# shaygong322/Mujoco-LIP-MPC-Simulation

Hardware: AMD Instinct MI355X
Metric: MPC solves/sec (batched scenarios), N=3 horizon 5-obstacle, 1->8 MI355X (higher is better)
Workload: dtype f64

## Files before the change

### mujoco-lip-mpc-simulation_amd/csrc/alipmpc.hip

```cpp
#include <hip/hip_runtime.h>

#include <atomic>
#include <cmath>
#include <cstdint>
#include <cstdio>
#include <cstdlib>
#include <cstring>
#include <map>
#include <mutex>
#include <string>
#include <type_traits>
#include <unordered_map>
#include <vector>

#include "../../include/alipmpc.h"

#ifndef ALIP_PART
#define ALIP_PART_HOST 1
#define ALIP_PART_N(k) 1
#else
#define ALIP_PART_HOST (ALIP_PART == 0)
#define ALIP_PART_N(k) (ALIP_PART == (k))
#endif

// ... 191 lines not shown
    static constexpr int NCP = 16 * NT;
    static constexpr int nu = 5 * N;
    static constexpr int NTU = (nu + 15) / 16;
    static constexpr int NCPU = 16 * NTU;
    static constexpr int NG = 8 * (N + 1);
    static constexpr int KLD = NCP + 1;
};

__device__ __forceinline__ int lane_id() { return threadIdx.x & (WAVE - 1); }

__device__ __forceinline__ void wave_sync()
{
    __builtin_amdgcn_wave_barrier();
    asm volatile("" ::: "memory");
}

__device__ __forceinline__ int rfl(int x) { return __builtin_amdgcn_readfirstlane(x); }
#define RELAUNDER(x) asm volatile("" : "+v"(x))

__device__ __forceinline__ double uni(double v)
{
    const int lo = __builtin_amdgcn_readfirstlane(__double2loint(v));
    const int hi = __builtin_amdgcn_readfirstlane(__double2hiint(v));
    return __hiloint2double(hi, lo);
}

__device__ __forceinline__ double bcast(double v, int src)
{
    int lo = __builtin_amdgcn_readlane(__double2loint(v), src);
    int hi = __builtin_amdgcn_readlane(__double2hiint(v), src);
    return __hiloint2double(hi, lo);
}

template <int CTRL>
__device__ __forceinline__ double dpp(double v)
{
    int lo = __builtin_amdgcn_update_dpp(0, __double2loint(v), CTRL, 0xF, 0xF, false);
    int hi = __builtin_amdgcn_update_dpp(0, __double2hiint(v), CTRL, 0xF, 0xF, false);
    return __hiloint2double(hi, lo);
}
__device__ __forceinline__ void swap16(double v, double& a, double& b)
{
    auto lo = __builtin_amdgcn_permlane16_swap((unsigned)__double2loint(v), (unsigned)__double2loint(v), false, false);
    auto hi = __builtin_amdgcn_permlane16_swap((unsigned)__double2hiint(v), (unsigned)__double2hiint(v), false, false);
    a = __hiloint2double((int)hi[0], (int)lo[0]);
    b = __hiloint2double((int)hi[1], (int)lo[1]);
}
__device__ __forceinline__ void swap32(double v, double& a, double& b)
{
    auto lo = __builtin_amdgcn_permlane32_swap((unsigned)__double2loint(v), (unsigned)__double2loint(v), false, false);
    auto hi = __builtin_amdgcn_permlane32_swap((unsigned)__double2hiint(v), (unsigned)__double2hiint(v), false, false);
    a = __hiloint2double((int)hi[0], (int)lo[0]);
    b = __hiloint2double((int)hi[1], (int)lo[1]);
}

__device__ __forceinline__ float uni(float v)
{
    return __int_as_float(__builtin_amdgcn_readfirstlane(__float_as_int(v)));
}
__device__ __forceinline__ float bcast(float v, int src)
{
    return __int_as_float(__builtin_amdgcn_readlane(__float_as_int(v), src));
}
template <int CTRL>
__device__ __forceinline__ float dpp(float v)
{
    return __int_as_float(__builtin_amdgcn_update_dpp(0, __float_as_int(v), CTRL, 0xF, 0xF, false));
}
__device__ __forceinline__ void swap16(float v, float& a, float& b)
{
    auto x = __builtin_amdgcn_permlane16_swap((unsigned)__float_as_int(v), (unsigned)__float_as_int(v), false, false);
    a = __int_as_float((int)x[0]);
    b = __int_as_float((int)x[1]);
}
__device__ __forceinline__ void swap32(float v, float& a, float& b)
{
    auto x = __builtin_amdgcn_permlane32_swap((unsigned)__float_as_int(v), (unsigned)__float_as_int(v), false, false);
    a = __int_as_float((int)x[0]);
    b = __int_as_float((int)x[1]);
}

struct OpAdd {
    template <class T>
    __device__ T operator()(T a, T b) const { return a + b; }
};
struct OpMax {
    template <class T>
    __device__ T operator()(T a, T b) const { return fmax(a, b); }
};
struct OpMin {
    template <class T>
    __device__ T operator()(T a, T b) const { return fmin(a, b); }
};

template <class T, class Op>
__device__ __forceinline__ T wreduce(T v, Op op)
{
    v = op(v, dpp<0xB1>(v));
    v = op(v, dpp<0x4E>(v));
    v = op(v, dpp<0x141>(v));
    v = op(v, dpp<0x140>(v));
    T a, b;
    swap16(v, a, b);
    v = op(a, b);
    swap32(v, a, b);
    return uni(op(a, b));
}
template <class T>
__device__ __forceinline__ T wsum(T v) { return wreduce(v, OpAdd()); }
template <class T>
__device__ __forceinline__ T wmax(T v) { return wreduce(v, OpMax()); }
template <class T>
__device__ __forceinline__ T wmin(T v) { return wreduce(v, OpMin()); }
template <class T>
__device__ __forceinline__ void wsum2(T& a, T& b)
{
    a = wsum(a);
    b = wsum(b);
}
template <class T>
__device__ __forceinline__ T gsum(T v)
{
    T a, b;
    swap16(v, a, b);
    v = a + b;
    swap32(v, a, b);
    return a + b;
}


__device__ __forceinline__ void ld4(const double* p, double& a, double& b, double& c, double& d)
{
    const double2* q = reinterpret_cast<const double2*>(p);
    const double2 x = q[0], y = q[1];
    a = x.x; b = x.y; c = y.x; d = y.y;
}
__device__ __forceinline__ void ld4(const float* p, float& a, float& b, float& c, float& d)
{
    const float4 x = *reinterpret_cast<const float4*>(p);
// ... 211 lines not shown
}

__device__ __forceinline__ int fexp2(double x) { return __builtin_amdgcn_frexp_exp(x); }
__device__ __forceinline__ int fexp2(float x) { return __builtin_amdgcn_frexp_expf(x); }

__device__ __forceinline__ double rsqrt_nr(double d)
{
    double y = __builtin_amdgcn_rsq(d);
    const double h = 0.5 * d;
    y = y * fma(-h * y, y, 1.5);
    y = y * fma(-h * y, y, 1.5);
    return y;
}
__device__ __forceinline__ double rcp_nr(double x)
{
    double y = __builtin_amdgcn_rcp(x);
    double e = fma(-x, y, 1.0);
    y = fma(y, e, y);
    e = fma(-x, y, 1.0);
    return fma(y, e, y);
}
__device__ __forceinline__ float rsqrt_nr(float d)
{
    float y = __builtin_amdgcn_rsqf(d);
    return y * fmaf(-0.5f * d * y, y, 1.5f);
}
__device__ __forceinline__ float rcp_nr(float x)
{
    float y = __builtin_amdgcn_rcpf(x);
    return fmaf(y, fmaf(-x, y, 1.0f), y);
}

#include "fastmath.inc"

template <int N, class WT>
__device__ void prologue(const KP& P, const WT& w, const typename WT::real* G, const double* E,
                         long long b, double& gxg, double& gyg, int& legv, double& uj)
{
    using D = Dim<N>;
    const int lane = lane_id();
    const double* x0 = P.x0 + 5 * b;
    legv = P.leg[b];
    const int ncr = P.nc[b];
    const int ner = P.ne ? P.ne[b] : 0;
    double x0v0 = x0[0], x0v1 = x0[1];
    double g0 = P.goal[2 * b], g1 = P.goal[2 * b + 1];
    {
        bool valid = lane < ncr && lane < P.nc_max;
        double c0 = 0, c1 = 0, c2 = 0;
        if (valid) {
            const double* c = P.cir + ((size_t)b * P.nc_max + lane) * 3;
            c0 = c[0]; c1 = c[1]; c2 = c[2];
        }
        double d = (x0v0 - c0) * (x0v0 - c0) + (x0v1 - c1) * (x0v1 - c1) - c2 * c2;
        bool keep = valid && (!P.select_obs || d <= P.detect_r2);
        unsigned long long m = __ballot(keep);
        int pos = __builtin_popcountll(m & ((1ull << lane) - 1ull));
        if (keep) {
            w.obs[3 * pos + 0] = c0;
            w.obs[3 * pos + 1] = c1;
            w.obs[3 * pos + 2] = c2;
        }
        if (lane == 0) w.nsel[0] = __builtin_popcountll(m);
    }
    if (P.ne_max > 0) {
        bool valid = lane < ner && lane < P.ne_max;
// ... 113 lines not shown
__device__ __forceinline__ bool gj_lds(R* M, int lane)
{
    constexpr int NE = n * (n + 1), Q = (NE + WAVE - 1) / WAVE;
    int ei[Q], ej[Q];
#pragma unroll
    for (int q = 0; q < Q; ++q) {
        const int e = lane + WAVE * q;
        ei[q] = e < NE ? e / (n + 1) : n;
        ej[q] = e < NE ? e - (e / (n + 1)) * (n + 1) : n;
    }
#pragma unroll 1
    for (int p = 0; p < n; ++p) {
        const R d = M[p * LD + p];
        R mip[Q], mpj[Q], mij[Q];
#pragma unroll
        for (int q = 0; q < Q; ++q) {
            mip[q] = M[ei[q] * LD + p];
            mpj[q] = M[p * LD + ej[q]];
            mij[q] = M[ei[q] * LD + ej[q]];
        }
        if (!(d > R(0))) return false;
        const R inv = rcp_nr(d);
#pragma unroll
        for (int q = 0; q < Q; ++q) {
            const R f = mpj[q] * inv;
            const R upd = ei[q] == p ? f : fma(-mip[q], f, mij[q]);
            M[ei[q] * LD + ej[q]] = ej[q] > p ? upd : mij[q];
        }
        wave_sync();
    }
    return true;
}

template <int n, class R>
__device__ __forceinline__ bool gj_regs(R (&a)[n + 1], int lane)
{
#pragma unroll
    for (int p = 0; p < n; ++p) {
        const R d = bcast(a[p], p);
        if (!(d > R(0))) return false;
        const R m = lane == p ? R(0) : a[p] * rcp_nr(d);
#pragma unroll
        for (int j = p + 1; j <= n; ++j) a[j] = fma(-m, bcast(a[j], p), a[j]);
    }
    R dg = a[0];
#pragma unroll
    for (int i = 1; i < n; ++i) dg = lane == i ? a[i] : dg;
    a[n] = a[n] * rcp_nr(dg);
    return true;
}

template <int n, int LDK, int LD, class R>
__device__ __forceinline__ void gj_fill(const R* K, R* M, int lane, R dw)
{
    constexpr int NE = n * (n + 1), Q = (NE + WAVE - 1) / WAVE;
#pragma unroll
    for (int q = 0; q < Q; ++q) {
        const int e = lane + WAVE * q;
        const int i = e < NE ? e / (n + 1) : n, j = e < NE ? e - (e / (n + 1)) * (n + 1) : n;
        const R v = e < NE ? K[i * LDK + j] : R(0);
        M[i * LD + j] = v + (i == j && e < NE ? dw : R(0));
    }
}
template <int n, int LD, class R>
__device__ __forceinline__ void gj_zero(R* M, int lane)
{
    constexpr int NE = n * (n + 1), Q = (NE + WAVE - 1) / WAVE;
#pragma unroll
    for (int q = 0; q < Q; ++q) {
        const int e = lane + WAVE * q;
        const int i = e < NE ? e / (n + 1) : n, j = e < NE ? e - (e / (n + 1)) * (n + 1) : n;
        M[i * LD + j] = R(0);
    }
}

template <int N, class R>
struct WSS {
    typedef R real;
    R* V;
    R* Vt;
    R* dV;
    R* CT;
// ... 753 lines not shown
#pragma unroll
                for (int T = 0; T < NT; ++T) {
                    const int cc = 16 * T + col;
                    const R j = ca.x * G[gen_i(pk, 0) * NCP + cc] + ca.y * G[gen_i(pk, 1) * NCP + cc] +
                                     cb.x * G[gen_i(pk, 2) * NCP + cc] + cb.y * G[gen_i(pk, 3) * NCP + cc];
                    gl[T] += j * y;
                    if constexpr (JC) jv[JC ? s : 0][T] = j;
                }
            }
#pragma unroll
            for (int T = 0; T < NT; ++T) gl[T] = gsum(gl[T]);
            STAMP(1);
            RELANE();
            R ru = R(0.0);
#pragma unroll
            for (int T = 0; T < NT; ++T)
                if (g4 == 0 && 16 * T + col < n) ru = fmax(ru, fabs(gl[T]));
            R rcm = R(0.0), nz = R(0.0), whi = -INFINITY, wlo = INFINITY;
#pragma unroll
            for (int q = 0; q < RPL; ++q) {
                const R dl = sr[q] - cl[q], du = cu[q] - sr[q];
                if (rtype[q] < R_NONE) rcm = fmax(rcm, fabs(cr[q] - sr[q]));
                nz += fabs(zl[q]) + fabs(zu[q]);
                if (HL(q)) {
                    whi = fmax(whi, dl * zl[q]);
                    wlo = fmin(wlo, dl * zl[q]);
                }
                if (HU(q)) {
                    whi = fmax(whi, du * zu[q]);
                    wlo = fmin(wlo, du * zu[q]);
                }
            }
            nz = wsum(nz);
            const R sd = uni(div100(fmax(R(100.0), rcp_div(nz, w.cst[K_MACT] + n))));
            const R sc = uni(div100(fmax(R(100.0), rcp_div(nz, fmax(R(1.0), w.cst[K_NBL])))));
            const R base_err = wmax(fmax(rcp_div(ru, sd), rcm));
            whi = wmax(whi);
            wlo = wmin(wlo);
            const bool anyw = whi >= wlo;
            const R comp0 = anyw ? fmax(fabs(whi), fabs(wlo)) : R(0.0);
            e0 = uni(fmax(base_err, rcp_div(comp0, sc)));
            if (rfl(P.goal_abort)) {
                bool at_goal = false;
#pragma unroll
                for (int q = 0; q < RPL; ++q) {
                    const R dxg = CK.gxg - rv[q][0], dyg = CK.gyg - rv[q][1];
                    at_goal |= rtype[q] == R_OBJ && dxg * dxg + dyg * dyg == R(0);
                }
                if (__ballot(at_goal) != 0ull) {
                    fail_it = it + FAIL_GOAL;
                    it_end = it;
                    break;
                }
            }
            if (e0 <= w.cst[K_TOL]) {
                status = 0;
                break;
            }
            if (it >= it_end) break;
            const R mu_min = w.cst[K_TOL] / R(11.0);
            const R mu_prev = mu;
            for (int t = 0; t < 8; ++t) {
                const R cm = anyw ? fmax(fabs(whi - mu), fabs(wlo - mu)) : R(0.0);
                if (fmax(base_err, rcp_div(cm, sc)) <= R(10.0) * mu && mu > mu_min)
                    mu = uni(fmax(mu_min, fmin(R(0.2) * mu, mu * sqrt(mu))));
                else
                    break;
            }
            if (mu != mu_prev) nf = 0;
            break;
        }
// ... 93 lines not shown
                }
            }
#pragma unroll
            for (int T = 0; T < NT; ++T) rhsc[T] = gsum(pw[T]);
#pragma unroll
            for (int i = 0; i < 4; ++i) {
                const int row = Mfma<R>::row(g4, i);
                w.K[row * KLD + col] = acc[0][0][i] + acc[1][0][i];
                if constexpr (NT == 2) {
                    const R k1 = acc[0][1][i] + acc[1][1][i];
                    w.K[row * KLD + 16 + col] = k1;
                    w.K[(16 + col) * KLD + row] = k1;
                    w.K[(16 + row) * KLD + 16 + col] = acc[0][2][i] + acc[1][2][i];
                }
            }
        }
        wave_sync();
        STAMP(4);
        RELANE();
        R xv;
        bool fact_ok = true;
        {
            R rhs_l = R(0.0);
#pragma unroll
            for (int T = 0; T < NT; ++T) rhs_l = (lane < n && (lane >> 4) == T) ? rhsc[T] : rhs_l;
            if constexpr (GJ && GJ_REGS) {
                R a[n + 1];
                auto fill = [&](R dw) {
#pragma unroll
                    for (int j = 0; j < n; ++j) a[j] = (lane < n ? w.K[lane * KLD + j] : R(0.0)) + (lane == j ? dw : R(0.0));
                    a[n] = rhs_l + R(0.0);
                };
                fill(R(0));
                if (!gj_regs<n>(a, lane)) {
                    R dw = dw_last == R(0.0) ? R(1e-4) : fmax(R(1e-20), dw_last / R(3.0));
                    for (;;) {
                        fill(dw);
                        if (gj_regs<n>(a, lane)) break;
                        dw *= dw_last == R(0.0) ? R(100.0) : R(8.0);
                        if (dw > R(sizeof(R) == 8 ? 1e40 : 1e30)) {
                            fact_ok = false;
                            break;
                        }
                    }
                    dw_last = uni(dw);
                }
                xv = lane < n ? a[n] : R(0.0);
            } else if constexpr (GJ) {
                if (lane < n) w.K[lane * KLD + n] = rhs_l;
                wave_sync();
                gj_fill<n, KLD, GJLD>(w.K, w.S, lane, R(0));
                wave_sync();
                if (!gj_lds<n, GJLD>(w.S, lane)) {
                    R dw = dw_last == R(0.0) ? R(1e-4) : fmax(R(1e-20), dw_last / R(3.0));
                    for (;;) {
                        gj_fill<n, KLD, GJLD>(w.K, w.S, lane, dw);
                        wave_sync();
                        if (gj_lds<n, GJLD>(w.S, lane)) break;
                        dw *= dw_last == R(0.0) ? R(100.0) : R(8.0);
                        if (dw > R(sizeof(R) == 8 ? 1e40 : 1e30)) {
                            fact_ok = false;
                            break;
                        }
                    }
                    dw_last = uni(dw);
                }
                xv = lane < n ? w.S[lane * GJLD + n] : R(0.0);
            } else {
                R a[n];
                R myidg = R(1.0);
#pragma unroll
// ... 11 lines not shown
                            fact_ok = false;
                            break;
                        }
                    }
                    dw_last = uni(dw);
                }
                R acc = R(0.0), yv = R(0.0);
#pragma unroll
                for (int k = 0; k < n; ++k) {
                    const R yk = bcast((rhs_l - acc) * myidg, k);
                    yv = lane == k ? yk : yv;
                    acc += lane > k ? a[k] * yk : R(0.0);
                }
                wave_sync();
                if (lane < n) {
#pragma unroll
                    for (int j = 0; j < n; ++j) w.K[lane * KLD + j] = j <= lane ? a[j] : R(0.0);
                }
                wave_sync();
                acc = R(0.0);
                xv = R(0.0);
#pragma unroll
                for (int i = n - 1; i >= 0; --i) {
                    const R xi = bcast((yv - acc) * myidg, i);
                    xv = lane == i ? xi : xv;
                    acc += lane < i ? w.K[i * KLD + (lane & 31)] * xi : R(0.0);
                }
            }
        }
        STAMP(5);
        RELANE();
        {
            R v = R(0.0);
#pragma unroll
            for (int j = 0; j < n; ++j)
                v += G[(lane < NG ? lane : 0) * NCP + j] * (GJ && !GJ_REGS ? w.S[j * GJLD + n] : bcast(xv, j));
            dvme = lane < NG && fact_ok ? v : R(0.0);
            if (lane < NG) w.dV[lane] = dvme;
        }
        wave_sync();
        if constexpr (GJ && !GJ_REGS) gj_zero<n, GJLD>(w.S, lane);
        if (!fact_ok && fail_it < 0) {
            fail_it = it;
            it_end = it + 1;
        }
        RELANE();
        R dS[RPL], dZl[RPL], dZu[RPL];
        R ap = R(1.0), az = R(1.0), theta = R(0.0), sl = R(0.0), jdv[RPL];
#pragma unroll
        for (int q = 0; q < RPL; ++q) {
            const int r = lane + WAVE * q;
#pragma unroll
            for (int i = 0; i < 4; ++i) rdv[q][i] = w.dV[gen_i(rg[q], i)];
            R jd = R(0.0);
            if (r < mo4) {
                struct { R x, y; } ca, cb;
                ld4(w.rcoef + 4 * r, ca.x, ca.y, cb.x, cb.y);
                jd = ca.x * rdv[q][0] + ca.y * rdv[q][1] + cb.x * rdv[q][2] + cb.y * rdv[q][3];
            }
            jdv[q] = jd;
            dS[q] = rtype[q] < R_NONE ? jd + rcv[q] : R(0.0);
            dZl[q] = HL(q) ? mu * idl[q] - zl[q] - zl[q] * idl[q] * dS[q] : R(0.0);
            dZu[q] = HU(q) ? mu * idu[q] - zu[q] + zu[q] * idu[q] * dS[q] : R(0.0);
            const R dl = sr[q] - cl[q], du = cu[q] - sr[q];
            const R ids = rcp_nr(dS[q]);
            if (HL(q) && dS[q] < 0) ap = fmin(ap, -tau * dl * ids);
            if (HU(q) && dS[q] > 0) ap = fmin(ap, tau * du * ids);
            if (HL(q) && dZl[q] < 0) az = fmin(az, -tau * zl[q] * rcp_nr(dZl[q]));
            if (HU(q) && dZu[q] < 0) az = fmin(az, -tau * zu[q] * rcp_nr(dZu[q]));
            theta += fabs(rcv[q]);
            sl += (HL(q) ? dS[q] * idl[q] : R(0.0)) - (HU(q) ? dS[q] * idu[q] : R(0.0));
        }
        ap = wmin(ap);
        az = wmin(az);
        theta = theta_ok ? theta_c : wsum(theta);
        const R gdv = obj_sum<N, RPL>(jdv, mr4);
        sl = wsum(sl);
        const R phi = uni(f_cur - mu * lsum_cur);
        const R gphi = uni(gdv - mu * sl);
        const R lsw = uni(gphi < 0 ? sth * llog(theta) - sph * llog(-gphi) : R(0.0));
        R amin;
        if (gphi < 0) {
            amin = fmin(gth, gph * theta / -gphi);
            if (theta <= w.cst[K_THMIN]) amin = fmin(amin, exp(lsw));
        } else {
            amin = gth;
        }
        amin *= gal;
        amin = uni(amin > R(0) ? amin : R(8.673617379884035e-19));
        STAMP(6);
        R a = ap;
        R la = uni(llog(ap));
        bool accepted = false, ftype = false;
        R ctr[RPL], ta0[RPL], ta1[RPL];
        R ft = R(0.0), lgt = R(0.0), tht_acc = R(0.0);
        bool redo = false;
        for (;;) {
            R am = a, lam = la;
            if (!(TM && redo))
                for (int t = 0; t < -1 - tm; ++t) {
                    am = uni(am * R(0.5));
                    lam = uni(lam - R(M_LN2));
                }
            const bool valid = am >= amin;
            bool acc_m = false, fty_m = false;
            if (valid) {
                WSTAMP_TRIAL;
                RELANE();
                R tht = R(0.0);
                ft = R(0.0);
                lgt = R(0.0);
                bool bad = false;
#pragma unroll
                for (int q = 0; q < RPL; ++q) {
                    R vt[4];
#pragma unroll
                    for (int i = 0; i < 4; ++i) vt[i] = fma(am, rdv[q][i], rv[q][i]);
                    R o[6];
#pragma unroll
                    for (int i = 0; i < 6; ++i) o[i] = w.obs6[6 * roi[q] + i];
                    row_trans(rtype[q], vt, w.cst[K_GXG], w.cst[K_GYG], ta0[q], ta1[q]);
                    ctr[q] = row_value(rtype[q], rk[q], vt, ta0[q], ta1[q], o, CK);
                    const R st = sr[q] + am * dS[q];
                    if (rtype[q] < R_NONE) tht += fabs(ctr[q] - st);

                    const R d1 = st - cl[q], d2 = cu[q] - st;
                    if (HL(q) && !(d1 > 0)) bad = true;
                    if (HU(q) && !(d2 > 0)) bad = true;
                    lgt += llog(HL(q) ? (HU(q) ? d1 * d2 : d1) : (HU(q) ? d2 : R(1.0)));
                }
                tht = wsum(tht);
                ft = obj_sum<N, RPL>(ctr, mr4);
                lgt = wsum(lgt);
                const bool anybad = __ballot(bad) != 0ull;
                const R pht = anybad ? INFINITY : ft - mu * lgt;
                bool ok = isfinite(pht) && tht < w.cst[K_THMAX];
                if (ok) {
                    const bool b0 = lane < nf && !(tht < fth0 || pht < fph0);
                    const bool b1 = lane + WAVE < nf && !(tht < fth1 || pht < fph1);
                    ok = __ballot(b0 || b1) == 0ull;
                }
                if (ok) {
                    const bool switching = gphi < 0 && lam > lsw;
                    if (switching && theta <= w.cst[K_THMIN]) {
                        if (pht <= phi + eta * am * gphi) {
                            acc_m = true;
                            fty_m = true;
                        }
                    } else if (tht <= (1 - gth) * theta || pht <= phi - gph * theta) {
                        acc_m = true;
                        fty_m = false;
                    }
                }
                tht_acc = tht;
            }
            if (TM && redo) {
                accepted = true;
                break;
            }
            if (!TM || tm >= 0) {
                if (!valid) break;
                if (acc_m) {
                    accepted = true;
                    ftype = fty_m;
                    break;
                }
// ... 2596 lines not shown
    using L = SweepL<NC, FEN>;
    auto kern = sweep_kernel<NC, FEN, CH, WPG>;
    const size_t smem = sizeof(double) * ((size_t)L::GL + (size_t)WPG * (CH / 2) * L::SLOTD);
    set_smem((const void*)kern, smem);
    const unsigned res = resident_blocks((const void*)kern, smem, WAVE * WPG);
    const long long per = (long long)CH * WPG;
    const unsigned need = (unsigned)((P.B + per - 1) / per);
    const unsigned grid = res > 0 && res < need ? res : (need > 0 ? need : 1u);
    hipLaunchKernelGGL(kern, dim3(grid), dim3(WAVE * WPG), smem, st, P);
}
template <int NC, bool FEN>
void launch_sweep_s(const KP& P, hipStream_t st)
{
    const char* se = getenv("ALIPMPC_SWEEP_SHAPE");
    const int shape = se ? atoi(se) : SWEEP_SHAPE_DEFAULT;
    if (shape == 641)
        launch_sweep_t<NC, FEN, 64, 1>(P, st);
    else
        launch_sweep_t<NC, FEN, 32, 2>(P, st);
}
hipError_t launch_sweep(int nc, bool fen, const KP& P, hipStream_t st)
{
#define SWCASE(K)                                              \
    case K:                                                    \
        fen ? launch_sweep_s<K, true>(P, st) : launch_sweep_s<K, false>(P, st); \
        break;
    switch (nc) {
        SWCASE(0) SWCASE(1) SWCASE(2) SWCASE(3) SWCASE(4) SWCASE(5) SWCASE(6)
    default:
        return hipErrorInvalidValue;
    }
#undef SWCASE
    return hipGetLastError();
}
#endif

}

#if ALIP_PART_HOST
#include "scenes.inc"
#include "dataset.inc"

namespace {

using namespace alip;

struct Handle {
    alipmpc_cfg cfg;
    int device = 0;
    int N = 3, n = 9, NG = 32, NCP = 16, NCPU = 16, rps = 0, m_max = 0, mr4 = 0;
    int rps_s = 0, m_s = 0, mr4_s = 0, mo4 = 0;
    double* dGp = nullptr;
    double* dEp = nullptr;
    double* dGu = nullptr;
    double* dEu = nullptr;
    double* dlk = nullptr;
    float* dlkf = nullptr;
    int lane_nct = -1;
    int sweep_nc = -1;
    static constexpr unsigned NQ = 64;
    uint32_t* dq = nullptr;
    mutable std::atomic<unsigned> qi{0};
    void* stage = nullptr;
    size_t stage_bytes = 0;
    void* rstage = nullptr;
    size_t rstage_bytes = 0;
// ... 1465 lines not shown
    return ALIPMPC_OK;
}

#ifdef ALIP_STAMPS
int alipmpc_dbg_stamps(unsigned long long* out, int reset)
{
    if (hipMemcpyFromSymbol(out, HIP_SYMBOL(alip::g_stamps), sizeof(unsigned long long) * alip::NSTAMP) != hipSuccess)
        return -1;
    if (reset) {
        unsigned long long z[alip::NSTAMP] = {};
        if (hipMemcpyToSymbol(HIP_SYMBOL(alip::g_stamps), z, sizeof(z)) != hipSuccess) return -1;
    }
    return alip::NSTAMP;
}
#endif

#ifdef ALIP_WSTAMP
int alipmpc_dbg_wstamps(unsigned long long* out, long long slots)
{
    if (slots > alip::WSTAMP_CAP) slots = alip::WSTAMP_CAP;
    if (hipDeviceSynchronize() != hipSuccess) return -1;
    if (hipMemcpyFromSymbol(out, HIP_SYMBOL(alip::g_wstamp), sizeof(unsigned long long) * 8 * (size_t)slots) != hipSuccess)
        return -1;
    const long long z = 0;
    if (hipMemcpyToSymbol(HIP_SYMBOL(alip::g_wstamp_base), &z, sizeof(z)) != hipSuccess) return -1;
    void* p = nullptr;
    if (hipGetSymbolAddress(&p, HIP_SYMBOL(alip::g_wstamp)) != hipSuccess ||
        hipMemset(p, 0, sizeof(unsigned long long) * 8 * (size_t)alip::WSTAMP_CAP) != hipSuccess)
        return -1;
    return (int)slots;
}
#endif

const char* alipmpc_build_id(void)
{
#ifdef ALIP_BUILD_ID
    return ALIP_BUILD_ID;
#else
    return "unknown";
#endif
}

double alipmpc_last_kernel_ms(void* handle)
{
    Handle* h = (Handle*)handle;
    if (!h || !h->timed) return 0.0;
    if (h->evlast < 0) return 0.0;
    hipEvent_t e0 = h->ev[h->evlast][0], e1 = h->ev[h->evlast][1];
    if (hipEventSynchronize(e1) != hipSuccess) return 0.0;
    float ms = 0.f;
    if (hipEventElapsedTime(&ms, e0, e1) != hipSuccess) return 0.0;
    return (double)ms;
}

const char* alipmpc_last_error(void* handle)
{
    Handle* h = (Handle*)handle;
    return h ? h->err.c_str() : "null handle";
}

int alipmpc_solve_slots(void* handle, int64_t* slots)
{
    Handle* h = (Handle*)handle;
    if (!h || !slots) return fail(h, ALIPMPC_EINVAL, "null argument");
    HIPCHK(h, hipSetDevice(h->device));
    unsigned res = 0;
// ... 92 lines not shown
```

### mujoco-lip-mpc-simulation_amd/csrc/resto_wave.inc

```
enum { RSW_OK = 0, RSW_INFEASIBLE = 1, RSW_MAXITER = 2, RSW_FAILED = 3 };

template <int N, int KSM, class R>
__device__ __forceinline__ int resto_wave(int wv, R fth0, R fph0, R fth1, R fph1, int nfo, R mu_o, R theta_R, int it)
{
    using D = Dim<N>;
    constexpr int n = D::n;
    constexpr int NT = D::NT;
    constexpr int NCP = D::NCP;
    constexpr int NG = D::NG;
    constexpr int KLD = D::KLD;
    constexpr int RPL = (4 * KSM + WAVE - 1) / WAVE;
    extern __shared__ __attribute__((aligned(16))) double smem[];
    const KP& P = *reinterpret_cast<const KP*>(smem);
    const R* G = reinterpret_cast<const R*>(smem + KP_DOUBLES);
    R* wsb = const_cast<R*>(G) + NG * NCP;
    int lane = lane_id();
    RSTAMP_DECL
    const int mr4 = rfl(P.mr4), mo4 = rfl(P.mo4), m_max = rfl(P.m_max), rps = rfl(P.rps);
    const int nc_max = rfl(P.nc_max), ne_max = rfl(P.ne_max), nobs = nc_max + ne_max;
    const int modi = rfl(P.modi), max_iter = rfl(P.max_iter);
    WSS<N, R> w = carve_s<N, R>(wsb + (size_t)wv * wss_elems<N, R>(nc_max, ne_max, mr4, mo4), nc_max, ne_max, mr4, mo4);
    const int nc_sel = w.nsel[0], ne_sel = w.nsel[1];
    const R rho = R(1000.0), tol = w.cst[K_TOL];
    const R gth = R(1e-5), gph = R(1e-8), sth = R(1.1), sph = R(2.3), eta = R(1e-8), gal = R(0.05);
// ... 69 lines not shown
        const R r_ = cr[q] - sr[q];
        const R a = (mu - rho * r_) / (R(2) * rho);
        const R sq = sqrt(a * a + mu * r_ / (R(2) * rho));
        const R nv = a >= R(0) ? a + sq : (mu * r_ / (R(2) * rho)) / (sq - a);
        nn[q] = isc ? nv : R(1);
        pp[q] = isc ? r_ + nv : R(1);
        zp[q] = isc ? mu / pp[q] : R(0);
        zn[q] = isc ? mu / nn[q] : R(0);
        vl[q] = isc && isfinite(cl[q]) ? fmin(rho, zl0[q]) : R(0);
        vu[q] = isc && isfinite(cu[q]) ? fmin(rho, zu0[q]) : R(0);
        yv[q] = R(0);
        if (isc) th0 += fabs(cr[q] - pp[q] + nn[q] - sr[q]);
    }
    th0 = wsum(th0);
    const R theta_max = R(1e4) * fmax(R(1), th0), theta_min = R(1e-4) * fmax(R(1), th0);
    R rft0 = INFINITY, rfp0 = INFINITY, rft1 = INFINITY, rfp1 = INFINITY;
    int nfr = 0;
    R dw_last = R(0);
    int code = RSW_OK;
    bool first = true;
    const int it_in = it;
    RSTAMP(0);
    for (;;) {
        RS_RELANE();
        R xc = lane < n ? w.V[gp(lane / 3, lane % 3)] : R(0);
        if (!first) {
            R tho = R(0), lso = R(0);
#pragma unroll
            for (int q = 0; q < RPL; ++q) {
                if (rtype[q] < R_NONE) tho += fabs(cr[q] - sr[q]);
                const R d1 = sr[q] - cl[q], d2_ = cu[q] - sr[q];
                lso += llog(isfinite(cl[q]) ? (isfinite(cu[q]) ? d1 * d2_ : d1) : (isfinite(cu[q]) ? d2_ : R(1.0)));
            }
            tho = wsum(tho);
            lso = wsum(lso);
            const R fo = obj_sum<N, RPL>(cr, mr4);
            const R pho = fo - mu_o * lso;
            bool acc = isfinite(pho) && tho <= R(0.9) * theta_R;
            if (acc) {
                const bool b0 = lane < nfo && !(tho < fth0 || pho < fph0);
                const bool b1 = lane + WAVE < nfo && !(tho < fth1 || pho < fph1);
                acc = __ballot(b0 || b1) == 0ull;
            }
            if (acc) {
                const R tau = uni(fmax(R(0.99), R(1) - mu_o));
                R dzl[RPL], dzu[RPL], ad = R(1);
#pragma unroll
                for (int q = 0; q < RPL; ++q) {
                    const bool hl = rtype[q] < R_NONE && isfinite(cl[q]), hu = rtype[q] < R_NONE && isfinite(cu[q]);
                    const R e1 = s0[q] - cl[q], e2 = cu[q] - s0[q];
                    dzl[q] = hl ? mu_o / e1 - zl0[q] - zl0[q] / e1 * (sr[q] - s0[q]) : R(0);
                    dzu[q] = hu ? mu_o / e2 - zu0[q] + zu0[q] / e2 * (sr[q] - s0[q]) : R(0);
                    if (hl && dzl[q] < R(0)) ad = fmin(ad, -tau * zl0[q] / dzl[q]);
                    if (hu && dzu[q] < R(0)) ad = fmin(ad, -tau * zu0[q] / dzu[q]);
                }
                ad = wmin(ad);
                R zmax = R(0);
#pragma unroll
                for (int q = 0; q < RPL; ++q) {
                    zl0[q] += ad * dzl[q];
                    zu0[q] += ad * dzu[q];
                    zmax = fmax(zmax, fmax(zl0[q], zu0[q]));
                }
                zmax = wmax(zmax);
                if (zmax > R(1000)) {
#pragma unroll
                    for (int q = 0; q < RPL; ++q) {
                        zl0[q] = rtype[q] < R_NONE && isfinite(cl[q]) ? R(1) : R(0);
// ... 49 lines not shown
                gl[T] += j * y;
            }
        }
#pragma unroll
        for (int T = 0; T < NT; ++T) gl[T] = gsum(gl[T]);
        R glme = gl[0];
#pragma unroll
        for (int T = 1; T < NT; ++T) glme = (lane >> 4) == T ? gl[T] : glme;
        RSTAMP(2);
        R zeta = uni(sqrt(mu));
        R gxv = lane < n ? zeta * d2 * (xc - xR) - glme : R(0);
        R dual = fabs(gxv), prim = R(0), nz = R(0), ny = R(0), whi = -INFINITY, wlo = INFINITY;
#pragma unroll
        for (int q = 0; q < RPL; ++q) {
            if (rtype[q] < R_NONE) {
                const R dl = sr[q] - cl[q], du = cu[q] - sr[q];
                dual = fmax(dual, fmax(fabs(rho + yv[q] - zp[q]), fabs(rho - yv[q] - zn[q])));
                dual = fmax(dual, fabs(yv[q] - vl[q] + vu[q]));
                prim = fmax(prim, fabs(cr[q] - pp[q] + nn[q] - sr[q]));
                ny += fabs(yv[q]);
                nz += fabs(zp[q]) + fabs(zn[q]) + fabs(vl[q]) + fabs(vu[q]);
                whi = fmax(whi, fmax(pp[q] * zp[q], nn[q] * zn[q]));
                wlo = fmin(wlo, fmin(pp[q] * zp[q], nn[q] * zn[q]));
                if (isfinite(cl[q])) {
                    whi = fmax(whi, dl * vl[q]);
                    wlo = fmin(wlo, dl * vl[q]);
                }
                if (isfinite(cu[q])) {
                    whi = fmax(whi, du * vu[q]);
                    wlo = fmin(wlo, du * vu[q]);
                }
            }
        }
        nz = wsum(nz);
        ny = wsum(ny);
        dual = wmax(dual);
        prim = wmax(prim);
        whi = wmax(whi);
        wlo = wmin(wlo);
        const R sd = uni(fmax(R(100), (nz + ny) / (R(n) + mal * R(3))) / R(100));
        const R sc = uni(fmax(R(100), nz / fmax(R(1), nbl)) / R(100));
        const R base = fmax(dual / sd, prim);
        const R e0 = uni(fmax(base, fmax(fabs(whi), fabs(wlo)) / sc));
        if (e0 <= tol) {
            R viol = R(0);
#pragma unroll
            for (int q = 0; q < RPL; ++q) {
                const int r = lane + WAVE * q;
                if (r < mr4 && rtype[q] < R_NONE) {
                    if (isfinite(cl[q])) viol = fmax(viol, w.rclo[r] - cr[q]);
                    if (isfinite(cu[q])) viol = fmax(viol, cr[q] - w.rcuo[r]);
                }
            }
            viol = wmax(viol);
            code = viol > R(1e-4) ? RSW_INFEASIBLE : RSW_OK;
            break;
        }
        if (it >= max_iter) {
            code = RSW_MAXITER;
            break;
        }
        const R mu_prev = mu;
        for (int t = 0; t < 8; ++t) {
            const R cm = fmax(fabs(whi - mu), fabs(wlo - mu));
            if (fmax(base, cm / sc) <= R(10) * mu && mu > tol / R(11))
                mu = uni(fmax(tol / R(11), fmin(R(0.2) * mu, mu * sqrt(mu))));
            else
                break;
        }
        if (mu != mu_prev) {
            nfr = 0;
            zeta = uni(sqrt(mu));
// ... 97 lines not shown
                }
            }
#pragma unroll
            for (int T = 0; T < NT; ++T) rhsc[T] = gsum(pw[T]);
#pragma unroll
            for (int i = 0; i < 4; ++i) {
                const int row = Mfma<R>::row(g4, i);
                w.K[row * KLD + col] = acc[0][0][i] + acc[1][0][i];
                if constexpr (NT == 2) {
                    const R k1 = acc[0][1][i] + acc[1][1][i];
                    w.K[row * KLD + 16 + col] = k1;
                    w.K[(16 + col) * KLD + row] = k1;
                    w.K[(16 + row) * KLD + 16 + col] = acc[0][2][i] + acc[1][2][i];
                }
            }
        }
        wave_sync();
        if (lane < n) w.K[lane * KLD + lane] += zeta * d2;
        wave_sync();
        R rhs_l = R(0);
#pragma unroll
        for (int T = 0; T < NT; ++T) rhs_l = (lane < n && (lane >> 4) == T) ? rhsc[T] : rhs_l;
        rhs_l = lane < n ? rhs_l - zeta * d2 * (xc - xR) : R(0);
        RSTAMP(6);
        R xv;
        if constexpr (n <= ALIP_GJ_MAX_N) {
            R a[n + 1];
            auto fill = [&](R dw) {
#pragma unroll
                for (int j = 0; j < n; ++j) a[j] = (lane < n ? w.K[lane * KLD + j] : R(0)) + (lane == j ? dw : R(0));
                a[n] = rhs_l + R(0);
            };
            fill(R(0));
            bool ok = gj_regs<n>(a, lane);
            if (!ok) {
                R dw = dw_last == R(0) ? R(1e-4) : fmax(R(1e-20), dw_last / R(3));
                for (;;) {
                    fill(dw);
                    if (gj_regs<n>(a, lane)) {
                        ok = true;
                        break;
                    }
                    dw *= dw_last == R(0) ? R(100) : R(8);
                    if (dw > R(sizeof(R) == 8 ? 1e40 : 1e30)) break;
                }
                dw_last = uni(dw);
            }
            if (!ok) {
                code = RSW_FAILED;
                break;
            }
            xv = lane < n ? a[n] : R(0);
        } else {
            R a[n];
            R myidg = R(1);
#pragma unroll
            for (int j = 0; j < n; ++j) a[j] = lane < n ? w.K[lane * KLD + j] : (lane == j ? R(1) : R(0));
            bool ok = chol_rows<n>(a, myidg, lane);
            if (!ok) {
                R dw = dw_last == R(0) ? R(1e-4) : fmax(R(1e-20), dw_last / R(3));
                for (;;) {
#pragma unroll
                    for (int j = 0; j < n; ++j)
                        a[j] = (lane < n ? w.K[lane * KLD + j] : (lane == j ? R(1) : R(0))) + (lane == j ? dw : R(0));
                    if (chol_rows<n>(a, myidg, lane)) {
                        ok = true;
                        break;
                    }
                    dw *= dw_last == R(0) ? R(100) : R(8);
                    if (dw > R(sizeof(R) == 8 ? 1e40 : 1e30)) break;
                }
                dw_last = uni(dw);
            }
            if (!ok) {
                code = RSW_FAILED;
                break;
            }
            R acc = R(0), yy = R(0);
#pragma unroll
            for (int k = 0; k < n; ++k) {
                const R yk = bcast((rhs_l - acc) * myidg, k);
                yy = lane == k ? yk : yy;
                acc += lane > k ? a[k] * yk : R(0);
            }
            wave_sync();
            if (lane < n) {
#pragma unroll
                for (int j = 0; j < n; ++j) w.K[lane * KLD + j] = j <= lane ? a[j] : R(0);
            }
            wave_sync();
            acc = R(0);
            xv = R(0);
#pragma unroll
            for (int i = n - 1; i >= 0; --i) {
                const R xi = bcast((yy - acc) * myidg, i);
                xv = lane == i ? xi : xv;
                acc += lane < i ? w.K[i * KLD + (lane & 31)] * xi : R(0);
            }
        }
        RS_RELANE();
        RSTAMP(7);
        {
            R v = R(0);
#pragma unroll
            for (int j = 0; j < n; ++j) v += G[(lane < NG ? lane : 0) * NCP + j] * bcast(xv, j);
            if (lane < NG) w.dV[lane] = v;
        }
        wave_sync();
        R dy[RPL], dpv[RPL], dnv[RPL], ds[RPL], dzp[RPL], dzn[RPL], dvl[RPL], dvu[RPL];
        R ap = R(1), az = R(1), theta = R(0), lin = R(0), gpn = R(0);
#pragma unroll
        for (int q = 0; q < RPL; ++q) {
            const int r = lane + WAVE * q;
#pragma unroll
            for (int i = 0; i < 4; ++i) rdv[q][i] = w.dV[gen_i(rg[q], i)];
            R jd = R(0);
            if (r < mo4) {
                R ca0, ca1, cb0, cb1;
                ld4(w.rcoef + 4 * r, ca0, ca1, cb0, cb1);
                jd = ca0 * rdv[q][0] + ca1 * rdv[q][1] + cb0 * rdv[q][2] + cb1 * rdv[q][3];
            }
            const bool isc = rtype[q] < R_NONE, hl = isc && isfinite(cl[q]), hu = isc && isfinite(cu[q]);
            const R dl = sr[q] - cl[q], du = cu[q] - sr[q];
            const R ipv = rcp_nr(pp[q]), inv = rcp_nr(nn[q]);
            const R idl_ = hl ? rcp_nr(dl) : R(0), idu_ = hu ? rcp_nr(du) : R(0);
            const R mdl = mu * idl_, mdu = mu * idu_;
            dy[q] = isc ? (bv[q] - jd) * iD[q] : R(0);
            dpv[q] = isc ? (-rho - yv[q] + mu * ipv - dy[q]) * iSp[q] : R(0);
            dnv[q] = isc ? (-rho + yv[q] + mu * inv + dy[q]) * iSn[q] : R(0);
            ds[q] = isc ? (-yv[q] + mdl - mdu - dy[q]) * iSs[q] : R(0);
            dzp[q] = isc ? mu * ipv - zp[q] - zp[q] * ipv * dpv[q] : R(0);
            dzn[q] = isc ? mu * inv - zn[q] - zn[q] * inv * dnv[q] : R(0);
            dvl[q] = hl ? mdl - vl[q] - vl[q] * idl_ * ds[q] : R(0);
            dvu[q] = hu ? mdu - vu[q] + vu[q] * idu_ * ds[q] : R(0);
            if (isc) {
                if (dpv[q] < R(0)) ap = fmin(ap, -tau * pp[q] * rcp_nr(dpv[q]));
                if (dnv[q] < R(0)) ap = fmin(ap, -tau * nn[q] * rcp_nr(dnv[q]));
                if (dzp[q] < R(0)) az = fmin(az, -tau * zp[q] * rcp_nr(dzp[q]));
                if (dzn[q] < R(0)) az = fmin(az, -tau * zn[q] * rcp_nr(dzn[q]));
                theta += fabs(cr[q] - pp[q] + nn[q] - sr[q]);
                gpn += (rho - mu * ipv) * dpv[q] + (rho - mu * inv) * dnv[q] - (mdl - mdu) * ds[q];
                lin += rho * (pp[q] + nn[q]) - mu * llog(pp[q] * nn[q] * (hl ? (hu ? dl * du : dl) : (hu ? du : R(1))));
            }
            const R ids = rcp_nr(ds[q]);
            if (hl && ds[q] < R(0)) ap = fmin(ap, -tau * dl * ids);
            if (hu && ds[q] > R(0)) ap = fmin(ap, tau * du * ids);
            if (hl && dvl[q] < R(0)) az = fmin(az, -tau * vl[q] * rcp_nr(dvl[q]));
            if (hu && dvu[q] < R(0)) az = fmin(az, -tau * vu[q] * rcp_nr(dvu[q]));
        }
        const R ex = lane < n ? xc - xR : R(0);
        lin += R(0.5) * zeta * d2 * ex * ex;
        gpn += zeta * d2 * ex * xv;
        ap = wmin(ap);
        az = wmin(az);
        theta = wsum(theta);
        const R gphi = wsum(gpn);
        const R phi = wsum(lin);
        R amin;
        if (gphi < R(0)) {
            amin = fmin(gth, gph * theta / -gphi);
            if (theta <= theta_min) amin = fmin(amin, exp(sth * llog(theta) - sph * llog(-gphi)));
        } else {
            amin = gth;
        }
        amin *= gal;
        amin = uni(amin > R(0) ? amin : R(8.673617379884035e-19));
        RSTAMP(8);
        R al = ap;
        bool accepted = false, ftype = false;
        R ctr[RPL], ta0[RPL], ta1[RPL];
        const R dxl = lane < n ? xv : R(0);
        while (al >= amin) {
            R tht = R(0), lt = R(0);
            bool bad = false;
#pragma unroll
            for (int q = 0; q < RPL; ++q) {
                R vt[4];
#pragma unroll
                for (int i = 0; i < 4; ++i) vt[i] = fma(al, rdv[q][i], rv[q][i]);
                R o[6];
#pragma unroll
                for (int i = 0; i < 6; ++i) o[i] = w.obs6[6 * roi[q] + i];
                row_trans(rtype[q], vt, w.cst[K_GXG], w.cst[K_GYG], ta0[q], ta1[q]);
                ctr[q] = row_value(rtype[q], rk[q], vt, ta0[q], ta1[q], o, RCK);
                if (rtype[q] < R_NONE) {
                    const R pt = pp[q] + al * dpv[q], nt = nn[q] + al * dnv[q], st = sr[q] + al * ds[q];
                    tht += fabs(ctr[q] - pt + nt - st);
                    const R d1 = st - cl[q], d2_ = cu[q] - st;
                    if (!(pt > R(0)) || !(nt > R(0))) bad = true;
                    if (isfinite(cl[q]) && !(d1 > R(0))) bad = true;
                    if (isfinite(cu[q]) && !(d2_ > R(0))) bad = true;
                    lt += rho * (pt + nt) -
                          mu * llog(pt * nt * (isfinite(cl[q]) ? (isfinite(cu[q]) ? d1 * d2_ : d1)
                                                               : (isfinite(cu[q]) ? d2_ : R(1))));
                }
            }
            const R et = ex + al * dxl;
            lt += R(0.5) * zeta * d2 * et * et;
            tht = wsum(tht);
            lt = wsum(lt);
            const R pht = __ballot(bad) != 0ull ? R(INFINITY) : lt;
            bool ok = isfinite(pht) && tht < theta_max;
            if (ok) {
                const bool b0 = lane < nfr && !(tht < rft0 || pht < rfp0);
                const bool b1 = lane + WAVE < nfr && !(tht < rft1 || pht < rfp1);
                ok = __ballot(b0 || b1) == 0ull;
            }
            if (ok) {
                const bool switching = gphi < R(0) && llog(al) + sph * llog(-gphi) > sth * llog(theta);
                if (switching && theta <= theta_min) {
                    if (pht <= phi + eta * al * gphi) {
                        accepted = true;
                        ftype = true;
                    }
                } else if (tht <= (R(1) - gth) * theta || pht <= phi - gph * theta) {
                    accepted = true;
                    ftype = false;
                }
            }
            if (accepted) break;
            al = uni(al * R(0.5));
        }
        RSTAMP(9);
        if (!accepted) {
            code = RSW_FAILED;
            break;
        }
        if (!ftype && nfr < FILTER_CAP) {
            const R fvt = (R(1) - gth) * theta, fvp = phi - gph * theta;
            if ((nfr & (WAVE - 1)) == lane) {
                if (nfr < WAVE) {
                    rft0 = fvt;
                    rfp0 = fvp;
                } else {
                    rft1 = fvt;
                    rfp1 = fvp;
                }
            }
            nfr++;
        }
        if (lane < NG) w.V[lane] = fma(al, w.dV[lane], w.V[lane]);
#pragma unroll
// ... 45 lines not shown
```

Measured before the change: 7.258 million.

## Pair wave reductions, use DPP row broadcasts, and pack scalar logs across lanes

Merges pairs of wave-wide reductions into one shared butterfly, with odd and even lanes carrying different values. Replaces readlane broadcasts in the register Gauss-Jordan elimination and the G·x products with DPP row_newbcast, and sets bound_ctrl on the DPP shuffles. Three scalar logs and the two error scales are now computed on different lanes at once and then broadcast. The goal is fewer cross-lane ops and less serial transcendental work in the IPM line search and factorisation. It also adds a debug kernel to check the new helpers, and the changes rely on the row-broadcast semantics being correct for n≤16.

```diff
diff --git a/mujoco-lip-mpc-simulation_amd/csrc/alipmpc.hip b/mujoco-lip-mpc-simulation_amd/csrc/alipmpc.hip
--- a/mujoco-lip-mpc-simulation_amd/csrc/alipmpc.hip
+++ b/mujoco-lip-mpc-simulation_amd/csrc/alipmpc.hip
@@ -247,11 +247,45 @@
     return __hiloint2double(hi, lo);
 }
 
+#ifdef ALIP_NO_RBCAST
+#define ALIP_RBCAST 0
+#else
+#define ALIP_RBCAST 1
+#endif
+#ifdef ALIP_NO_WRED2
+#define ALIP_WRED2 0
+#else
+#define ALIP_WRED2 1
+#endif
+#ifdef ALIP_NO_DPP_BC
+constexpr bool DPP_BC = false;
+#else
+constexpr bool DPP_BC = true;
+#endif
+#ifdef ALIP_NO_PACKF
+#define ALIP_PACKF 0
+#else
+#define ALIP_PACKF 1
+#endif
+
+template <int P>
+__device__ __forceinline__ double rbcast(double v)
+{
+    static_assert(P >= 0 && P < 16, "row_newbcast selects a lane of the row");
+    return __builtin_amdgcn_update_dpp(0.0, v, 0x150 + P, 0xF, 0xF, true);
+}
+template <int P>
+__device__ __forceinline__ float rbcast(float v)
+{
+    static_assert(P >= 0 && P < 16, "row_newbcast selects a lane of the row");
+    return __int_as_float(__builtin_amdgcn_update_dpp(0, __float_as_int(v), 0x150 + P, 0xF, 0xF, true));
+}
+
 template <int CTRL>
 __device__ __forceinline__ double dpp(double v)
 {
-    int lo = __builtin_amdgcn_update_dpp(0, __double2loint(v), CTRL, 0xF, 0xF, false);
-    int hi = __builtin_amdgcn_update_dpp(0, __double2hiint(v), CTRL, 0xF, 0xF, false);
+    int lo = __builtin_amdgcn_update_dpp(0, __double2loint(v), CTRL, 0xF, 0xF, DPP_BC);
+    int hi = __builtin_amdgcn_update_dpp(0, __double2hiint(v), CTRL, 0xF, 0xF, DPP_BC);
     return __hiloint2double(hi, lo);
 }
 __device__ __forceinline__ void swap16(double v, double& a, double& b)
@@ -280,7 +314,7 @@
 template <int CTRL>
 __device__ __forceinline__ float dpp(float v)
 {
-    return __int_as_float(__builtin_amdgcn_update_dpp(0, __float_as_int(v), CTRL, 0xF, 0xF, false));
+    return __int_as_float(__builtin_amdgcn_update_dpp(0, __float_as_int(v), CTRL, 0xF, 0xF, DPP_BC));
 }
 __device__ __forceinline__ void swap16(float v, float& a, float& b)
 {
@@ -320,6 +354,46 @@
     v = op(a, b);
     swap32(v, a, b);
     return uni(op(a, b));
+}
+template <class T, class Op>
+__device__ __forceinline__ void wreduce2(T& a, T& b, Op op)
+{
+#if ALIP_WRED2
+    const bool odd = (lane_id() & 1) != 0;
+    const T keep = odd ? b : a, give = odd ? a : b;
+    T v = op(keep, dpp<0xB1>(give));
+    v = op(v, dpp<0x4E>(v));
+    v = op(v, dpp<0x12C>(v));
+    v = op(v, dpp<0x128>(v));
+    T x, y;
+    swap16(v, x, y);
+    v = op(x, y);
+    swap32(v, x, y);
+    v = op(x, y);
+    a = bcast(v, 0);
+    b = bcast(v, 1);
+#else
+    a = wreduce(a, op);
+    b = wreduce(b, op);
+#endif
+}
+template <class T>
+__device__ __forceinline__ void wsum_pair(T& a, T& b) { wreduce2(a, b, OpAdd()); }
+template <class T>
+__device__ __forceinline__ void wmax_pair(T& a, T& b) { wreduce2(a, b, OpMax()); }
+template <class T>
+__device__ __forceinline__ void wmin_pair(T& a, T& b) { wreduce2(a, b, OpMin()); }
+template <class T>
+__device__ __forceinline__ void wmaxmin_pair(T& hi, T& lo)
+{
+#if ALIP_WRED2
+    T nlo = -lo;
+    wreduce2(hi, nlo, OpMax());
+    lo = -nlo;
+#else
+    hi = wreduce(hi, OpMax());
+    lo = wreduce(lo, OpMin());
+#endif
 }
 template <class T>
 __device__ __forceinline__ T wsum(T v) { return wreduce(v, OpAdd()); }
@@ -597,6 +671,34 @@
 }
 
 #include "fastmath.inc"
+
+template <class T>
+__device__ __forceinline__ void llog3(T x0, T x1, T x2, T& l0, T& l1, T& l2)
+{
+#if ALIP_PACKF
+    const int l = lane_id();
+    const T r = llog(l == 0 ? x0 : (l == 1 ? x1 : x2));
+    l0 = bcast(r, 0);
+    l1 = bcast(r, 1);
+    l2 = bcast(r, 2);
+#else
+    l0 = uni(llog(x0));
+    l1 = uni(llog(x1));
+    l2 = uni(llog(x2));
+#endif
+}
+template <class T>
+__device__ __forceinline__ void err_scales(T nz, T den0, T den1, T& sd, T& sc)
+{
+#if ALIP_PACKF
+    const T r = div100(fmax(T(100.0), rcp_div(nz, lane_id() == 1 ? den1 : den0)));
+    sd = bcast(r, 0);
+    sc = bcast(r, 1);
+#else
+    sd = uni(div100(fmax(T(100.0), rcp_div(nz, den0))));
+    sc = uni(div100(fmax(T(100.0), rcp_div(nz, den1))));
+#endif
+}
 
 template <int N, class WT>
 __device__ void prologue(const KP& P, const WT& w, const typename WT::real* G, const double* E,
@@ -776,22 +878,57 @@
     return true;
 }
 
-template <int n, class R>
-__device__ __forceinline__ bool gj_regs(R (&a)[n + 1], int lane)
-{
-#pragma unroll
-    for (int p = 0; p < n; ++p) {
+template <int RPL>
+constexpr bool gj_rb = ALIP_RBCAST != 0 && RPL == 1;
+template <int p, int n, bool RB, class R>
+__device__ __forceinline__ bool gj_steps(R (&a)[n + 1], int lane)
+{
+    if constexpr (p < n) {
         const R d = bcast(a[p], p);
         if (!(d > R(0))) return false;
         const R m = lane == p ? R(0) : a[p] * rcp_nr(d);
 #pragma unroll
-        for (int j = p + 1; j <= n; ++j) a[j] = fma(-m, bcast(a[j], p), a[j]);
-    }
+        for (int j = p + 1; j <= n; ++j) {
+            if constexpr (RB && sizeof(R) == 8)
+                a[j] = fma(-m, rbcast<p>(a[j]), a[j]);
+            else
+                a[j] = fma(-m, bcast(a[j], p), a[j]);
+        }
+        return gj_steps<p + 1, n, RB>(a, lane);
+    } else {
+        return true;
+    }
+}
+template <int n, class R, bool RB>
+__device__ __forceinline__ bool gj_regs(R (&a)[n + 1], int lane)
+{
+    static_assert(n <= 16, "the rows sit in one 16-lane row");
+    if (!gj_steps<0, n, RB>(a, lane)) return false;
     R dg = a[0];
 #pragma unroll
     for (int i = 1; i < n; ++i) dg = lane == i ? a[i] : dg;
     a[n] = a[n] * rcp_nr(dg);
     return true;
+}
+
+template <int n, int NG, class R>
+constexpr bool dp_rows = ALIP_RBCAST != 0 && sizeof(R) == 8 && n <= 16 && NG <= 32;
+template <int j, int n, class R>
+__device__ __forceinline__ R gdp_acc(const R* Grow, R x, R v)
+{
+    if constexpr (j < n) {
+        v += Grow[j] * rbcast<j>(x);
+        return gdp_acc<j + 1, n>(Grow, x, v);
+    } else {
+        return v;
+    }
+}
+template <int n, int NCP, class R>
+__device__ __forceinline__ R gdp_rows(const R* G, R xv, int t)
+{
+    R x0, x1;
+    swap16(xv, x0, x1);
+    return gdp_acc<0, n>(G + t * NCP, x0, R(0.0));
 }
 
 template <int n, int LDK, int LD, class R>
@@ -1611,11 +1748,10 @@
                 }
             }
             nz = wsum(nz);
-            const R sd = uni(div100(fmax(R(100.0), rcp_div(nz, w.cst[K_MACT] + n))));
-            const R sc = uni(div100(fmax(R(100.0), rcp_div(nz, fmax(R(1.0), w.cst[K_NBL])))));
+            R sd, sc;
+            err_scales(nz, w.cst[K_MACT] + n, fmax(R(1.0), w.cst[K_NBL]), sd, sc);
             const R base_err = wmax(fmax(rcp_div(ru, sd), rcm));
-            whi = wmax(whi);
-            wlo = wmin(wlo);
+            wmaxmin_pair(whi, wlo);
             const bool anyw = whi >= wlo;
             const R comp0 = anyw ? fmax(fabs(whi), fabs(wlo)) : R(0.0);
             e0 = uni(fmax(base_err, rcp_div(comp0, sc)));
@@ -1775,11 +1911,11 @@
                     a[n] = rhs_l + R(0.0);
                 };
                 fill(R(0));
-                if (!gj_regs<n>(a, lane)) {
+                if (!gj_regs<n, R, gj_rb<RPL>>(a, lane)) {
                     R dw = dw_last == R(0.0) ? R(1e-4) : fmax(R(1e-20), dw_last / R(3.0));
                     for (;;) {
                         fill(dw);
-                        if (gj_regs<n>(a, lane)) break;
+                        if (gj_regs<n, R, gj_rb<RPL>>(a, lane)) break;
                         dw *= dw_last == R(0.0) ? R(100.0) : R(8.0);
                         if (dw > R(sizeof(R) == 8 ? 1e40 : 1e30)) {
                             fact_ok = false;
@@ -1857,9 +1993,13 @@
         RELANE();
         {
             R v = R(0.0);
-#pragma unroll
-            for (int j = 0; j < n; ++j)
-                v += G[(lane < NG ? lane : 0) * NCP + j] * (GJ && !GJ_REGS ? w.S[j * GJLD + n] : bcast(xv, j));
+            if constexpr (GJ && GJ_REGS && dp_rows<n, NG, R>) {
+                v = gdp_rows<n, NCP>(G, xv, lane < NG ? lane : 0);
+            } else {
+#pragma unroll
+                for (int j = 0; j < n; ++j)
+                    v += G[(lane < NG ? lane : 0) * NCP + j] * (GJ && !GJ_REGS ? w.S[j * GJLD + n] : bcast(xv, j));
+            }
             dvme = lane < NG && fact_ok ? v : R(0.0);
             if (lane < NG) w.dV[lane] = dvme;
         }
@@ -1896,14 +2036,15 @@
             theta += fabs(rcv[q]);
             sl += (HL(q) ? dS[q] * idl[q] : R(0.0)) - (HU(q) ? dS[q] * idu[q] : R(0.0));
         }
-        ap = wmin(ap);
-        az = wmin(az);
+        wmin_pair(ap, az);
         theta = theta_ok ? theta_c : wsum(theta);
         const R gdv = obj_sum<N, RPL>(jdv, mr4);
         sl = wsum(sl);
         const R phi = uni(f_cur - mu * lsum_cur);
         const R gphi = uni(gdv - mu * sl);
-        const R lsw = uni(gphi < 0 ? sth * llog(theta) - sph * llog(-gphi) : R(0.0));
+        R lth, lgp, lap;
+        llog3(theta, -gphi, ap, lth, lgp, lap);
+        const R lsw = uni(gphi < 0 ? sth * lth - sph * lgp : R(0.0));
         R amin;
         if (gphi < 0) {
             amin = fmin(gth, gph * theta / -gphi);
@@ -1915,7 +2056,7 @@
         amin = uni(amin > R(0) ? amin : R(8.673617379884035e-19));
         STAMP(6);
         R a = ap;
-        R la = uni(llog(ap));
+        R la = lap;
         bool accepted = false, ftype = false;
         R ctr[RPL], ta0[RPL], ta1[RPL];
         R ft = R(0.0), lgt = R(0.0), tht_acc = R(0.0);
@@ -1954,9 +2095,8 @@
                     if (HU(q) && !(d2 > 0)) bad = true;
                     lgt += llog(HL(q) ? (HU(q) ? d1 * d2 : d1) : (HU(q) ? d2 : R(1.0)));
                 }
-                tht = wsum(tht);
+                wsum_pair(tht, lgt);
                 ft = obj_sum<N, RPL>(ctr, mr4);
-                lgt = wsum(lgt);
                 const bool anybad = __ballot(bad) != 0ull;
                 const R pht = anybad ? INFINITY : ft - mu * lgt;
                 bool ok = isfinite(pht) && tht < w.cst[K_THMAX];
@@ -4619,6 +4759,71 @@
     }
 #undef SWCASE
     return hipGetLastError();
+}
+#endif
+
+#if ALIP_PART_HOST
+constexpr int WH_SET = 32 + 2 * 16 * WAVE;
+template <int P>
+__device__ __forceinline__ void wh_bcasts(double a, double* o, int lane)
+{
+    if constexpr (P < 16) {
+        const double r0 = bcast(a, P), r1 = bcast(a, 16 + P), r2 = bcast(a, 32 + P), r3 = bcast(a, 48 + P);
+        o[WAVE * P + lane] = lane < 16 ? r0 : (lane < 32 ? r1 : (lane < 48 ? r2 : r3));
+        o[16 * WAVE + WAVE * P + lane] = rbcast<P>(a);
+        wh_bcasts<P + 1>(a, o, lane);
+    }
+}
+__global__ __launch_bounds__(WAVE) void wave_helpers_kernel(const double* in, int nsets, const double* sys, int nsys,
+                                                            double* out, double* gj_out)
+{
+    const int lane = lane_id();
+    for (int s = 0; s < nsets; ++s) {
+        const double a = in[2 * WAVE * s + lane], b = in[2 * WAVE * s + WAVE + lane];
+        double* o = out + (size_t)WH_SET * s;
+        double r[26];
+        r[0] = wreduce(a, OpAdd()); r[1] = wreduce(b, OpAdd());
+        r[2] = wreduce(a, OpMax()); r[3] = wreduce(b, OpMax());
+        r[4] = wreduce(a, OpMin()); r[5] = wreduce(b, OpMin());
+        r[6] = a; r[7] = b;
+        wsum_pair(r[6], r[7]);
+        r[8] = a; r[9] = b;
+        wmax_pair(r[8], r[9]);
+        r[10] = a; r[11] = b;
+        wmin_pair(r[10], r[11]);
+        r[12] = wreduce(a, OpMax()); r[13] = wreduce(b, OpMin());
+        r[14] = a; r[15] = b;
+        wmaxmin_pair(r[14], r[15]);
+        const double a0 = bcast(a, 0), a1 = bcast(a, 1), a2 = bcast(a, 2);
+        r[16] = uni(llog(a0)); r[17] = uni(llog(a1)); r[18] = uni(llog(a2));
+        llog3(a0, a1, a2, r[19], r[20], r[21]);
+        const double nz = bcast(b, 0), d0 = bcast(b, 1), d1 = bcast(b, 2);
+        r[22] = uni(div100(fmax(100.0, rcp_div(nz, d0))));
+        r[23] = uni(div100(fmax(100.0, rcp_div(nz, d1))));
+        err_scales(nz, d0, d1, r[24], r[25]);
+        double mine = 0.0;
+#pragma unroll
+        for (int i = 0; i < 26; ++i) mine = lane == i ? r[i] : mine;
+        if (lane < 26) o[lane] = mine;
+        wh_bcasts<0>(a, o + 32, lane);
+    }
+    for (int m = 0; m < nsys; ++m) {
+        constexpr int n = 9;
+        double a[n + 1], c[n + 1];
+#pragma unroll
+        for (int j = 0; j <= n; ++j) a[j] = c[j] = lane < n ? sys[(n + 1) * (n * m + lane) + j] : 0.0;
+        const bool ok_a = gj_regs<n, double, false>(a, lane);
+        const bool ok_c = gj_regs<n, double, true>(c, lane);
+        double* o = gj_out + 2 * (n + 1) * m;
+        if (lane < n) {
+            o[lane] = a[n];
+            o[n + 1 + lane] = c[n];
+        }
+        if (lane == n) {
+            o[n] = ok_a ? 1.0 : 0.0;
+            o[2 * n + 1] = ok_c ? 1.0 : 0.0;
+        }
+    }
 }
 #endif
 
@@ -6150,6 +6355,27 @@
 }
 #endif
 
+int alipmpc_dbg_wave_helpers(const double* in, int nsets, const double* sys, int nsys, double* out, double* gj_out)
+{
+    if (nsets < 0 || nsys < 0 || nsets > 4096 || nsys > 4096) return -1;
+    const size_t zi = sizeof(double) * 2 * alip::WAVE * (size_t)nsets, zs = sizeof(double) * 90 * (size_t)nsys;
+    const size_t zo = sizeof(double) * alip::WH_SET * (size_t)nsets, zg = sizeof(double) * 20 * (size_t)nsys;
+    double* d = nullptr;
+    if (hipMalloc((void**)&d, zi + zs + zo + zg + 8) != hipSuccess) return -1;
+    double *di = d, *ds = di + 2 * alip::WAVE * (size_t)nsets, *dout = ds + 90 * (size_t)nsys,
+           *dg = dout + alip::WH_SET * (size_t)nsets;
+    bool ok = (zi == 0 || hipMemcpy(di, in, zi, hipMemcpyHostToDevice) == hipSuccess) &&
+              (zs == 0 || hipMemcpy(ds, sys, zs, hipMemcpyHostToDevice) == hipSuccess);
+    if (ok) {
+        hipLaunchKernelGGL(alip::wave_helpers_kernel, dim3(1), dim3(alip::WAVE), 0, 0, di, nsets, ds, nsys, dout, dg);
+        ok = hipGetLastError() == hipSuccess && hipDeviceSynchronize() == hipSuccess &&
+             (zo == 0 || hipMemcpy(out, dout, zo, hipMemcpyDeviceToHost) == hipSuccess) &&
+             (zg == 0 || hipMemcpy(gj_out, dg, zg, hipMemcpyDeviceToHost) == hipSuccess);
+    }
+    hipFree(d);
+    return ok ? alip::WH_SET : -1;
+}
+
 const char* alipmpc_build_id(void)
 {
 #ifdef ALIP_BUILD_ID
diff --git a/mujoco-lip-mpc-simulation_amd/csrc/resto_wave.inc b/mujoco-lip-mpc-simulation_amd/csrc/resto_wave.inc
--- a/mujoco-lip-mpc-simulation_amd/csrc/resto_wave.inc
+++ b/mujoco-lip-mpc-simulation_amd/csrc/resto_wave.inc
@@ -125,8 +125,7 @@
                 const R d1 = sr[q] - cl[q], d2_ = cu[q] - sr[q];
                 lso += llog(isfinite(cl[q]) ? (isfinite(cu[q]) ? d1 * d2_ : d1) : (isfinite(cu[q]) ? d2_ : R(1.0)));
             }
-            tho = wsum(tho);
-            lso = wsum(lso);
+            wsum_pair(tho, lso);
             const R fo = obj_sum<N, RPL>(cr, mr4);
             const R pho = fo - mu_o * lso;
             bool acc = isfinite(pho) && tho <= R(0.9) * theta_R;
@@ -242,12 +241,9 @@
                 }
             }
         }
-        nz = wsum(nz);
-        ny = wsum(ny);
-        dual = wmax(dual);
-        prim = wmax(prim);
-        whi = wmax(whi);
-        wlo = wmin(wlo);
+        wsum_pair(nz, ny);
+        wmax_pair(dual, prim);
+        wmaxmin_pair(whi, wlo);
         const R sd = uni(fmax(R(100), (nz + ny) / (R(n) + mal * R(3))) / R(100));
         const R sc = uni(fmax(R(100), nz / fmax(R(1), nbl)) / R(100));
         const R base = fmax(dual / sd, prim);
@@ -411,12 +407,12 @@
                 a[n] = rhs_l + R(0);
             };
             fill(R(0));
-            bool ok = gj_regs<n>(a, lane);
+            bool ok = gj_regs<n, R, gj_rb<RPL>>(a, lane);
             if (!ok) {
                 R dw = dw_last == R(0) ? R(1e-4) : fmax(R(1e-20), dw_last / R(3));
                 for (;;) {
                     fill(dw);
-                    if (gj_regs<n>(a, lane)) {
+                    if (gj_regs<n, R, gj_rb<RPL>>(a, lane)) {
                         ok = true;
                         break;
                     }
@@ -481,8 +477,12 @@
         RSTAMP(7);
         {
             R v = R(0);
-#pragma unroll
-            for (int j = 0; j < n; ++j) v += G[(lane < NG ? lane : 0) * NCP + j] * bcast(xv, j);
+            if constexpr (dp_rows<n, NG, R>) {
+                v = gdp_rows<n, NCP>(G, xv, lane < NG ? lane : 0);
+            } else {
+#pragma unroll
+                for (int j = 0; j < n; ++j) v += G[(lane < NG ? lane : 0) * NCP + j] * bcast(xv, j);
+            }
             if (lane < NG) w.dV[lane] = v;
         }
         wave_sync();
@@ -530,10 +530,9 @@
         const R ex = lane < n ? xc - xR : R(0);
         lin += R(0.5) * zeta * d2 * ex * ex;
         gpn += zeta * d2 * ex * xv;
-        ap = wmin(ap);
-        az = wmin(az);
-        theta = wsum(theta);
-        const R gphi = wsum(gpn);
+        wmin_pair(ap, az);
+        wsum_pair(theta, gpn);
+        const R gphi = gpn;
         const R phi = wsum(lin);
         R amin;
         if (gphi < R(0)) {
@@ -576,8 +575,7 @@
             }
             const R et = ex + al * dxl;
             lt += R(0.5) * zeta * d2 * et * et;
-            tht = wsum(tht);
-            lt = wsum(lt);
+            wsum_pair(tht, lt);
             const R pht = __ballot(bad) != 0ull ? R(INFINITY) : lt;
             bool ok = isfinite(pht) && tht < theta_max;
             if (ok) {
@@ -586,7 +584,12 @@
                 ok = __ballot(b0 || b1) == 0ull;
             }
             if (ok) {
-                const bool switching = gphi < R(0) && llog(al) + sph * llog(-gphi) > sth * llog(theta);
+                bool switching = false;
+                if (gphi < R(0)) {
+                    R lal, lgp, lth;
+                    llog3(al, -gphi, theta, lal, lgp, lth);
+                    switching = lal + sph * lgp > sth * lth;
+                }
                 if (switching && theta <= theta_min) {
                     if (pht <= phi + eta * al * gphi) {
                         accepted = true;
```

Result: faster. 7.825 million, median of 6 (+7.8%).
